# ComparativeGenomicsToolkit/cactus

Hardware: NVIDIA H100
Metric: BAR POA DP Gcells/sec and ends/sec at 1/2/4/8 H100 vs reference CPU BAR (higher is better)
Workload: dtype int32

## Files before the change

### cactus_b200/csrc/poa_cta.cuh

```cuda
#pragma once
#include <cuda_runtime.h>
#include "poa_graph.cuh"

namespace barb200 {

__device__ int cta_excl_scan(int *a, int n, int *ws) {
    const int T = blockDim.x, tid = threadIdx.x, lane = tid & 31, warp = tid >> 5, nw = T >> 5;
    const int chunk = (n + T - 1) / T, b = min(n, tid * chunk), e = min(n, b + chunk);
    int s = 0;
    for (int i = b; i < e; ++i) s += a[i];
    int inc = s;
#pragma unroll
    for (int off = 1; off < 32; off <<= 1) { const int v = __shfl_up_sync(0xffffffffu, inc, off); if (lane >= off) inc += v; }
    __syncthreads();
    if (lane == 31) ws[warp] = inc;
    __syncthreads();
    int woff = 0, total = 0;
    for (int k = 0; k < nw; ++k) { const int v = ws[k]; if (k < warp) woff += v; total += v; }
    int run = woff + inc - s;
    for (int i = b; i < e; ++i) { const int v = a[i]; a[i] = run; run += v; }
    __syncthreads();
    return total;
}

__device__ void cta_incl_max_scan(int *a, int n, int *ws) {
    const int T = blockDim.x, tid = threadIdx.x, lane = tid & 31, warp = tid >> 5, nw = T >> 5;
    const int chunk = (n + T - 1) / T, b = min(n, tid * chunk), e = min(n, b + chunk);
    int s = INT32_MIN;
    for (int i = b; i < e; ++i) s = max(s, a[i]);
    int inc = s;
#pragma unroll
    for (int off = 1; off < 32; off <<= 1) { const int v = __shfl_up_sync(0xffffffffu, inc, off); if (lane >= off) inc = max(inc, v); }
    int run = __shfl_up_sync(0xffffffffu, inc, 1);
    if (lane == 0) run = INT32_MIN;
    __syncthreads();
    if (lane == 31) ws[warp] = inc;
    __syncthreads();
    for (int k = 0; k < nw; ++k) if (k < warp) run = max(run, ws[k]);
    for (int i = b; i < e; ++i) { run = max(run, a[i]); a[i] = run; }
    __syncthreads();
}

__device__ __forceinline__ bool grow_in_par(Graph &g, int t) {
    if (g.in_n[t] < g.in_cap[t]) return true;
    const int ncap = g.in_cap[t] ? g.in_cap[t] * 2 : 2;
    const int noff = atomicAdd(&g.in_used, ncap);
    if (noff + ncap > g.in_pool) { g.err = JOB_ERR_EDGE_CAP; return false; }
    for (int i = 0; i < g.in_n[t]; ++i) { g.in_id[noff + i] = g.in_id[g.in_off[t] + i]; g.in_w[noff + i] = g.in_w[g.in_off[t] + i]; }
    g.in_off[t] = noff; g.in_cap[t] = ncap;
    return true;
}
__device__ __forceinline__ bool grow_out_par(Graph &g, int f) {
    if (g.out_n[f] < g.out_cap[f]) return true;
    const int ncap = g.out_cap[f] ? g.out_cap[f] * 2 : 2;
    const int noff = atomicAdd(&g.out_used, ncap);
    if (noff + ncap > g.out_pool) { g.err = JOB_ERR_EDGE_CAP; return false; }
    const int W = g.W;
    for (int i = 0; i < g.out_n[f]; ++i) {
        g.out_id[noff + i] = g.out_id[g.out_off[f] + i]; g.out_w[noff + i] = g.out_w[g.out_off[f] + i];
        for (int w = 0; w < W; ++w) g.out_rid[(int64_t)(noff + i) * W + w] = g.out_rid[(int64_t)(g.out_off[f] + i) * W + w];
    }
    for (int i = g.out_n[f]; i < ncap; ++i) for (int w = 0; w < W; ++w) g.out_rid[(int64_t)(noff + i) * W + w] = 0;
    g.out_off[f] = noff; g.out_cap[f] = ncap;
    return true;
}
__device__ __forceinline__ void graph_add_edge_par(Graph &g, int from, int to, int check_edge, int read_id) {
    int out_i = -1;
    if (check_edge) {
        const int io = g.in_off[to], in = g.in_n[to];
        for (int i = 0; i < in; ++i) if (g.in_id[io + i] == from) { g.in_w[io + i] += 1; break; }
        const int oo = g.out_off[from], on = g.out_n[from];
        for (int i = 0; i < on; ++i) if (g.out_id[oo + i] == to) { g.out_w[oo + i] += 1; out_i = i; break; }
    }
    if (out_i < 0) {
        if (!grow_in_par(g, to) || !grow_out_par(g, from)) return;
        const int ip = g.in_off[to] + g.in_n[to]; g.in_id[ip] = from; g.in_w[ip] = 1; g.in_n[to]++;
        out_i = g.out_n[from];
        const int op = g.out_off[from] + out_i; g.out_id[op] = to; g.out_w[op] = 1; g.out_n[from]++;
    }
    g.out_rid[(int64_t)(g.out_off[from] + out_i) * g.W + (read_id >> 6)] |= 1ULL << (read_id & 63);
}

__device__ void cta_add_first_sequence(Graph &g, const uint8_t *seq, int len, int read_id) {
    const int tid = threadIdx.x, T = blockDim.x, W = g.W;
    if (len + 2 > g.node_cap) { if (tid == 0) g.err = JOB_ERR_NODE_CAP; __syncthreads(); return; }
    if (2 * (len + 1) > g.in_pool || 2 * (len + 1) > g.out_pool) { if (tid == 0) g.err = JOB_ERR_EDGE_CAP; __syncthreads(); return; }
    const int rw = read_id >> 6; const uint64_t rb = 1ULL << (read_id & 63);
    for (int i = tid; i <= len; i += T) {
        const int to = i < len ? 2 + i : SINK_ID, from = i == 0 ? SRC_ID : 1 + i;
        g.in_off[to] = 2 * i; g.in_n[to] = 1; g.in_cap[to] = 2; g.in_id[2 * i] = from; g.in_w[2 * i] = 1;
        g.out_off[from] = 2 * i; g.out_n[from] = 1; g.out_cap[from] = 2; g.out_id[2 * i] = to; g.out_w[2 * i] = 1;
        for (int w = 0; w < W; ++w) { g.out_rid[(int64_t)(2 * i) * W + w] = w == rw ? rb : 0; g.out_rid[(int64_t)(2 * i + 1) * W + w] = 0; }
        if (i < len) { g.base[to] = seq[i]; g.aln_n[to] = 0; }
        g.index_to_node[i + 1] = to; g.node_to_index[to] = i + 1;
    }
    if (tid == 0) { g.index_to_node[0] = SRC_ID; g.node_to_index[SRC_ID] = 0; }
    if (tid == 0) { g.node_n = len + 2; g.in_used = 2 * (len + 1); g.out_used = 2 * (len + 1); }
    __syncthreads();
}

__device__ void cta_fuse_alignment(Graph &g, const uint8_t *seq, int L, const uint64_t *cigar, int n_cigar, int read_id, int *ws) {
    const int tid = threadIdx.x, T = blockDim.x;
    if (n_cigar == 0) return;
    int *node_of = g.tmp0, *is_new = g.tmp1;
    for (int c = tid; c < n_cigar; c += T) {
        const uint64_t cg = cigar[c];
        const int op = (int)(cg & 0xf);
        if (op == CMATCH) {
            const int node_id = (int)((cg >> 34) & 0x3fffffff), q = (int)((cg >> 4) & 0x3fffffff);
            const uint8_t b = seq[q];
            if (g.base[node_id] == b) { node_of[q] = node_id; is_new[q] = 0; }
            else {
                const int a = graph_aligned_with_base(g, node_id, b);
                if (a != -1) { node_of[q] = a; is_new[q] = 0; } else { node_of[q] = -1 - node_id; is_new[q] = 1; }
            }
        } else if (op == CINS) {
            const int qe = (int)((cg >> 34) & 0x3fffffff), len = (int)((cg >> 4) & 0x3fffffff);
            for (int q = qe - len + 1; q <= qe; ++q) { node_of[q] = INT32_MIN; is_new[q] = 1; }
        }
    }
    __syncthreads();
    const int first_new = g.node_n;
    const int n_new = cta_excl_scan(is_new, L, ws);
    if (first_new + n_new > g.node_cap) { if (tid == 0) g.err = JOB_ERR_NODE_CAP; __syncthreads(); return; }
    for (int q = tid; q < L; q += T) {
        const int m = node_of[q];
        if (m >= 0) { is_new[q] = 0; continue; }
        const int nid = first_new + is_new[q];
        g.base[nid] = seq[q]; g.aln_n[nid] = 0;
        g.in_off[nid] = 0; g.in_n[nid] = 0; g.in_cap[nid] = 0; g.out_off[nid] = 0; g.out_n[nid] = 0; g.out_cap[nid] = 0;
        if (m != INT32_MIN) graph_add_aligned(g, -1 - m, nid);
        node_of[q] = nid; is_new[q] = 1;
    }
    if (tid == 0) g.node_n = first_new + n_new;
    __syncthreads();
    if (g.err) return;
    {
        int *anc = g.remain, *cnt = g.msa_rank, *new_i2n = g.tmp1;
        const int n_old = first_new;
        for (int q = tid; q < L; q += T) {
            const int v = node_of[q];
            int e = v < first_new ? g.node_to_index[v] : -1;
            for (int k = 0; k < g.aln_n[v]; ++k) { const int a = g.aln_id[v * 4 + k]; if (a < first_new) e = max(e, g.node_to_index[a]); }
            anc[q] = e;
        }
        for (int i = tid; i < n_old; i += T) cnt[i] = 0;
        __syncthreads();
        cta_incl_max_scan(anc, L, ws);
        for (int q = tid; q < L; q += T) if (node_of[q] >= first_new) atomicAdd(&cnt[max(anc[q], 0)], 1);
        __syncthreads();
        cta_excl_scan(cnt, n_old, ws);
        for (int i = tid; i < n_old; i += T) new_i2n[i + cnt[i]] = g.index_to_node[i];
        for (int q = tid; q < L; q += T) { const int v = node_of[q]; if (v >= first_new) new_i2n[max(anc[q], 0) + 1 + (v - first_new)] = v; }
        __syncthreads();
        for (int k = tid; k < first_new + n_new; k += T) { const int v = new_i2n[k]; g.index_to_node[k] = v; g.node_to_index[v] = k; }
        __syncthreads();
    }
    for (int q = tid; q <= L; q += T) {
        const int from = q == 0 ? SRC_ID : node_of[q - 1], to = q == L ? SINK_ID : node_of[q];
        const int fresh = (q > 0 && from >= first_new) || (q < L && to >= first_new);
        graph_add_edge_par(g, from, to, fresh ? 0 : 1, read_id);
    }
    __syncthreads();
}


__device__ __forceinline__ void prefetch_l2(const void *p) { asm volatile("prefetch.global.L2 [%0];" ::"l"(p)); }

__device__ int warp_backtrack_step(const RowTables &rt, const DpState &d, const PoaParams &P, const int *smat8, const uint8_t *q,
                                   int &i, int &j, int &cur_op, int &len) {
    const unsigned FULLM = 0xffffffffu;
    const int lane = threadIdx.x & 31, inf = P.inf_min, e1 = P.e1, e2 = P.e2, oe1 = P.o1 + P.e1, oe2 = P.o2 + P.e2;
    len = 1;
    const RowRec rc = rt.rec[i];
    const RowInfo ri = d.info[i];
    const int *rowi = d.planes + d.row_off[i];
    const int npre = rc.base_npre >> 8;
    const int s = smat8[8 * (rc.base_npre & 0xff) + q[j - 1]];
    int hij = inf; unsigned cij = (unsigned)E_NEG16 | (unsigned)E_NEG16 << 16;
    if (j >= ri.beg && j <= ri.end) { hij = __ldcg(rowi + plane_index(ri.beg, ri.end, 0, j)); cij = (unsigned)__ldcg(rowi + plane_index(ri.beg, ri.end, 1, j)); }
    int hk0 = inf;
    if ((cur_op & OP_F) && j - 1 - lane >= ri.beg && j - 1 - lane <= ri.end) hk0 = __ldcg(rowi + plane_index(ri.beg, ri.end, 0, j - 1 - lane));
    int pi = -1, pm = inf, ph = inf, pe1 = inf, pe2 = inf; bool m_in = false, e_in = false;
    auto probe = [&](int kb) {
        const int k = kb + lane;
        pi = -1; m_in = false; e_in = false;
        if (k >= npre) return;
        pi = k == 0 ? rc.pre0 : rt.pre_row[rc.pre_off + k];
        const RowInfo pin = d.info[pi];
        const int *prow = d.planes + d.row_off[pi];
        m_in = (cur_op & OP_M) && j - 1 >= pin.beg && j - 1 <= pin.end;
        e_in = (cur_op & OP_E) && j >= pin.beg && j <= pin.end;
        if (m_in) pm = __ldcg(prow + plane_index(pin.beg, pin.end, 0, j - 1));
        if (e_in) {
            ph = __ldcg(prow + plane_index(pin.beg, pin.end, 0, j));
            const unsigned code = (unsigned)__ldcg(prow + plane_index(pin.beg, pin.end, 1, j));
            pe1 = e_decode(ph, (int)(code & 0xffffu), inf); pe2 = e_decode(ph, (int)(code >> 16), inf);
        }
    };
    if (cur_op & OP_M) {
        for (int kb = 0; kb < npre; kb += 32) {
            probe(kb);
            const unsigned hit = __ballot_sync(FULLM, m_in && pm + s == hij);
            if (hit) { i = __shfl_sync(FULLM, pi, __ffs(hit) - 1); --j; cur_op = OP_ALL; return CMATCH; }
        }
    }
    if (cur_op & OP_E) {
        const int own_e1 = e_decode(hij, (int)(cij & 0xffffu), inf), own_e2 = e_decode(hij, (int)(cij >> 16), inf);
        for (int kb = 0; kb < npre; kb += 32) {
            if (npre > 32 || !(cur_op & OP_M)) probe(kb);
            const bool ok1 = e_in && (cur_op & OP_E1) && ((cur_op & OP_M) ? hij == pe1 : own_e1 == pe1 - e1);
            const bool ok2 = e_in && (cur_op & OP_E2) && ((cur_op & OP_M) ? hij == pe2 : own_e2 == pe2 - e2);
            const unsigned hit = __ballot_sync(FULLM, ok1 || ok2);
            if (hit) {
                const int f = __ffs(hit) - 1;
                const int nop = ok1 ? ((ph - oe1 == pe1) ? (OP_M | OP_F) : OP_E1) : ((ph - oe2 == pe2) ? (OP_M | OP_F) : OP_E2);
                cur_op = __shfl_sync(FULLM, nop, f); i = __shfl_sync(FULLM, pi, f);
                return CDEL;
            }
        }
    }
    if (cur_op & OP_F) {
        if (!(cur_op & OP_M)) return -1;
        const int avail = j - ri.beg;
        int t1_max;
        if (e1 > e2) t1_max = oe2 >= oe1 ? (oe2 - oe1) / (e1 - e2) + 1 : 0;
        else t1_max = (e1 < e2 || oe1 <= oe2) ? avail : 0;
        if (t1_max > avail) t1_max = avail;
        for (int which = 0; which < 2; ++which) {
            if (!(cur_op & (which ? OP_F2 : OP_F1))) continue;
            const int oe = which ? oe2 : oe1, e = which ? e2 : e1, tmax = which ? avail : t1_max;
            for (int t0 = 0; t0 < tmax; t0 += 32) {
                const int t = t0 + lane + 1;
                int hk = hk0;
                if (t0 > 0) { hk = inf; if (t <= avail) hk = __ldcg(rowi + plane_index(ri.beg, ri.end, 0, j - t)); }
                const unsigned hit = __ballot_sync(FULLM, t <= tmax && hk == hij + oe + (t - 1) * e);
                if (hit) { len = __ffs(hit); len += t0; j -= len; cur_op = OP_M | OP_E; return CINS; }
            }
        }
    }
    return -1;
}

__device__ void warp_backtrack(Graph &g, const RowTables &rt, DpState &d, const PoaParams &P, const int *smat8, const uint8_t *q, int L) {
    const unsigned FULLM = 0xffffffffu;
    const int lane = threadIdx.x & 31, inf = P.inf_min;
    if (lane == 0) { dp_best_cell(g, rt, d, P, L); d.fc_row = -1; d.fc_hi = -1; }
    __syncwarp();
    int i = d.best_i, j = d.best_j, cur_op = OP_ALL, nc = 0, last_op = -1;
    uint64_t *cg = d.cigar; const int cap = d.cigar_cap;
    int fail = 0;
    auto push = [&](int op, int len, int node_id, int query_id) {
        if (nc == 0 || op != CINS || last_op != CINS) {
            if (nc >= cap) { fail = JOB_ERR_CIGAR_CAP; return; }
            if (lane == 0) {
                const uint64_t n_id = (uint64_t)(int64_t)node_id, q_id = (uint64_t)(int64_t)query_id, l = (uint64_t)len;
                cg[nc] = op == CMATCH ? (n_id << 34 | q_id << 4 | (uint64_t)op) : op == CINS ? (q_id << 34 | l << 4 | (uint64_t)op) : (n_id << 34 | l << 4 | (uint64_t)op);
            }
            ++nc;
        } else if (lane == 0) cg[nc - 1] += (uint64_t)len << 4;
        last_op = op;
    };
    if (j < L) push(CINS, L - j, -1, L - 1);
#ifdef BT_PROFILE
    long long pf_t0 = clock64(), pf_run_t = 0, pf_step_t = 0; int pf_iters = 0, pf_runs = 0, pf_cells = 0, pf_steps = 0, pf_ins = 0;
#endif
    while (i > 0 && j > 0 && !fail) {
        int run = 0;
#ifdef BT_PROFILE
        long long pf_a = clock64();
#endif
        if (cur_op == OP_ALL) {
            int c = i - lane, pre = -1, base = 0, n_ok = 0, node = 0;
            RowInfo ric; ric.beg = 0; ric.end = -1; ric.left = 0; ric.right = 0;
            int64_t ro = 0;
            bool fresh = true;
#pragma unroll 1
            for (int it = 0; it < 4; ++it) {
                if (fresh) {
                    pre = -1;
                    if (c > 0) { const RowRec rc = rt.rec[c]; base = rc.base_npre & 0xff; pre = (rc.base_npre >> 8) ? rc.pre0 : -1; node = g.index_to_node[c]; }
                    if (c >= 0) { ric = d.info[c]; ro = d.row_off[c]; }
                }
                const int nxt = __shfl_down_sync(FULLM, c, 1);
                const bool ok = lane < 31 && pre >= 0 && pre == nxt;
                n_ok = __ffs(~__ballot_sync(FULLM, ok)) - 1;
                if (n_ok >= 31 || it == 3) break;
                const int pre_b = __shfl_sync(FULLM, pre, n_ok);
                if (pre_b < 0) break;
                fresh = lane > n_ok;
                if (fresh) c = pre_b - (lane - n_ok - 1);
            }
            const int jj = j - lane;
            int hv = inf, inb = 0;
            if (lane <= n_ok && c >= 0 && jj >= 0) {
                inb = jj >= ric.beg && jj <= ric.end;
                if (inb) hv = __ldcg(d.planes + ro + plane_index(ric.beg, ric.end, 0, jj));
            }
            const int cl = c - 32, jl = jj - 32;
            RowInfo ril; ril.beg = 0; ril.end = -1; ril.left = 0; ril.right = 0;
            int64_t rol = 0;
            if (cl >= 0 && jl >= 0) { ril = d.info[cl]; rol = d.row_off[cl]; prefetch_l2(rt.rec + cl); prefetch_l2(g.index_to_node + cl); }
            const int h_next = __shfl_down_sync(FULLM, hv, 1), inb_next = __shfl_down_sync(FULLM, inb, 1);
            bool hit = false;
            if (lane < n_ok && c > 0 && jj >= 1 && inb_next) hit = h_next + smat8[8 * base + q[jj - 1]] == hv;
            run = __ffs(~__ballot_sync(FULLM, hit)) - 1;
            if (run > 0) {
                if (nc + run > cap) fail = JOB_ERR_CIGAR_CAP;
                else {
                    if (lane < run) cg[nc + lane] = (uint64_t)node << 34 | (uint64_t)(jj - 1) << 4 | (uint64_t)CMATCH;
                    nc += run; last_op = CMATCH;
                    i = __shfl_sync(FULLM, c, run); j -= run;
                }
            }
            if (cl >= 0 && jl >= 0 && jl <= ril.end) prefetch_l2(d.planes + rol + plane_index(ril.beg, ril.end, 0, jl < ril.beg ? ril.beg : jl));
        }
#ifdef BT_PROFILE
        long long pf_b = clock64(); if (cur_op == OP_ALL) { pf_run_t += pf_b - pf_a; ++pf_iters; if (run) { ++pf_runs; pf_cells += run; } }
#endif
        if (run == 0 && !fail) {
            const int id = g.index_to_node[i], jq = j - 1;
            int len = 1;
            const int op = warp_backtrack_step(rt, d, P, smat8, q, i, j, cur_op, len);
            if (op < 0) fail = JOB_ERR_BACKTRACK; else push(op, len, id, jq);
#ifdef BT_PROFILE
            pf_step_t += clock64() - pf_b; ++pf_steps; if (op == CINS) ++pf_ins;
#endif
        }
    }
#ifdef BT_PROFILE
    if (lane == 0 && blockIdx.x == 0) printf("bt L=%d total=%lld run_t=%lld step_t=%lld iters=%d runs=%d cells=%d steps=%d ins=%d\n", L, clock64() - pf_t0, pf_run_t, pf_step_t, pf_iters, pf_runs, pf_cells, pf_steps, pf_ins);
#endif
    if (!fail && j > 0) push(CINS, j, -1, j - 1);
    if (fail) { if (lane == 0) g.err = fail; return; }
    if (lane == 0) d.n_cigar = nc;
    __syncwarp();
    for (int a = lane; a < nc >> 1; a += 32) { const uint64_t t = cg[a]; cg[a] = cg[nc - 1 - a]; cg[nc - 1 - a] = t; }
    __syncwarp();
}

struct BfsScratch { uint32_t *optr; uint16_t *odst, *queue, *indeg; uint8_t *alnn; };

__device__ __forceinline__ size_t bfs_scratch_bytes(int n, int E) { return (size_t)4 * (n + 1) + (size_t)2 * E + 4 * (size_t)n + n + 16; }

__device__ void bfs_index_smem(Graph &g, const BfsScratch &B) {
    const int n = g.node_n;
    int head = 0, tail = 0;
    B.queue[tail++] = SRC_ID;
    while (head < tail) {
        const int cur = B.queue[head++];
        if (cur == SINK_ID) {
            if (head != n) g.err = JOB_ERR_TOPO;
            return;
        }
        const uint32_t o0 = B.optr[cur], o1 = B.optr[cur + 1];
        for (uint32_t i = o0; i < o1; ++i) {
            const int o = B.odst[i];
            const int left = (int)B.indeg[o] - 1; B.indeg[o] = (uint16_t)left;
            if (left == 0) {
                const int an = B.alnn[o];
                bool ok = true;
                for (int j = 0; j < an; ++j) if (B.indeg[g.aln_id[o * 4 + j]] != 0) { ok = false; break; }
                if (!ok) continue;
                B.queue[tail++] = (uint16_t)o;
                for (int j = 0; j < an; ++j) B.queue[tail++] = (uint16_t)g.aln_id[o * 4 + j];
            }
        }
    }
    g.err = JOB_ERR_TOPO;
}

__device__ void cta_topo_sort(Graph &g, RowTables &rt, unsigned char *scr, int scr_bytes, int *ws, bool have_order) {
    const int tid = threadIdx.x, T = blockDim.x, n = g.node_n;
    if (have_order) {
        for (int v = tid; v < n; v += T) graph_sort_node_edges(g, v);
        __syncthreads();
    } else {
    for (int v = tid; v < n; v += T) g.tmp0[v] = g.out_n[v];
    __syncthreads();
    const int E = cta_excl_scan(g.tmp0, n, ws);
    if (n < 65536 && bfs_scratch_bytes(n, E) <= (size_t)scr_bytes) {
        BfsScratch B;
        B.optr = reinterpret_cast<uint32_t *>(scr);
        B.odst = reinterpret_cast<uint16_t *>(B.optr + n + 1);
        B.queue = B.odst + E; B.indeg = B.queue + n;
        B.alnn = reinterpret_cast<uint8_t *>(B.indeg + n);
        for (int v = tid; v < n; v += T) {
            const uint32_t o = (uint32_t)g.tmp0[v];
            B.optr[v] = o;
            const int oo = g.out_off[v], on = g.out_n[v];
            for (int i = 0; i < on; ++i) B.odst[o + i] = (uint16_t)g.out_id[oo + i];
            B.indeg[v] = (uint16_t)g.in_n[v]; B.alnn[v] = g.aln_n[v];
        }
        if (tid == 0) B.optr[n] = (uint32_t)E;
        __syncthreads();
        if (T > 32) {
            if (tid == 0) bfs_index_smem(g, B);
            else if (tid >= 32) for (int v = tid - 32; v < n; v += T - 32) graph_sort_node_edges(g, v);
        } else {
            if (tid == 0) bfs_index_smem(g, B);
            __syncwarp();
            for (int v = tid; v < n; v += T) graph_sort_node_edges(g, v);
        }
        __syncthreads();
        if (g.err) return;
        for (int k = tid; k < n; k += T) { const int v = B.queue[k]; g.index_to_node[k] = v; g.node_to_index[v] = k; }
    } else {
        if (tid == 0) graph_bfs_index(g);
        __syncthreads();
        if (g.err) return;
        for (int v = tid; v < n; v += T) graph_sort_node_edges(g, v);
    }
    __syncthreads();
    }
    int *nx[2] = {g.tmp0, g.tmp1}, *dd[2] = {g.remain, g.msa_rank};
    for (int v = tid; v < n; v += T) {
        int nxt = SINK_ID, dist = 0;
        if (v != SINK_ID) {
            int max_w = -1;
            const int oo = g.out_off[v], on = g.out_n[v];
            for (int i = 0; i < on; ++i) if (g.out_w[oo + i] > max_w) { max_w = g.out_w[oo + i]; nxt = g.out_id[oo + i]; }
            dist = 1;
        }
        nx[0][v] = nxt; dd[0][v] = dist;
    }
    __syncthreads();
    int cur = 0;
    for (int span = 1; span < n; span <<= 1, cur ^= 1) {
        for (int v = tid; v < n; v += T) {
            const int nv = nx[cur][v];
            dd[cur ^ 1][v] = dd[cur][v] + dd[cur][nv];
            nx[cur ^ 1][v] = nx[cur][nv];
        }
        __syncthreads();
    }
    if (cur == 0) { for (int v = tid; v < n; v += T) g.remain[v] -= 1; }
    else { for (int v = tid; v < n; v += T) g.remain[v] = g.msa_rank[v] - 1; }
    __syncthreads();
    for (int r = tid; r < n; r += T) g.tmp0[r] = g.in_n[g.index_to_node[r]];
    __syncthreads();
    cta_excl_scan(g.tmp0, n, ws);
    for (int r = tid; r < n; r += T) graph_build_row(g, rt, r, g.tmp0[r]);
    __syncthreads();
}


__device__ void cta_msa_rank(Graph &g, unsigned char *scr, int scr_bytes, int *ws, int *msa_len_out) {
    const int tid = threadIdx.x, T = blockDim.x, n = g.node_n;
    for (int v = tid; v < n; v += T) g.tmp0[v] = g.out_n[v];
    __syncthreads();
    const int E = cta_excl_scan(g.tmp0, n, ws);
    if (n < 65535 && bfs_scratch_bytes(n, E) + 2 * (size_t)n <= (size_t)scr_bytes) {
        BfsScratch B;
        B.optr = reinterpret_cast<uint32_t *>(scr);
        B.odst = reinterpret_cast<uint16_t *>(B.optr + n + 1);
        B.queue = B.odst + E; B.indeg = B.queue + n;
        uint16_t *rk = B.indeg + n;
        B.alnn = reinterpret_cast<uint8_t *>(rk + n);
        for (int v = tid; v < n; v += T) {
            const uint32_t o = (uint32_t)g.tmp0[v];
            B.optr[v] = o;
            const int oo = g.out_off[v], on = g.out_n[v];
            for (int i = 0; i < on; ++i) B.odst[o + i] = (uint16_t)g.out_id[oo + i];
            B.indeg[v] = (uint16_t)g.in_n[v]; B.alnn[v] = g.aln_n[v];
        }
        if (tid == 0) B.optr[n] = (uint32_t)E;
        __syncthreads();
        if (tid == 0) {
            uint16_t *st = B.queue;
            int sp = 0, rank = 0, len = -1;
            st[sp++] = SRC_ID; rk[SRC_ID] = 0xffff;
            while (sp > 0) {
                const int cur = st[--sp];
                if (rk[cur] == 0xffff) {
                    rk[cur] = (uint16_t)rank;
                    for (int i = 0; i < B.alnn[cur]; ++i) rk[g.aln_id[cur * 4 + i]] = (uint16_t)rank;
                    ++rank;
                }
                if (cur == SINK_ID) { len = (int)rk[SINK_ID] - 1; break; }
                const uint32_t o0 = B.optr[cur], o1 = B.optr[cur + 1];
                for (uint32_t i = o0; i < o1; ++i) {
                    const int o = B.odst[i];
                    const int left = (int)B.indeg[o] - 1; B.indeg[o] = (uint16_t)left;
                    if (left == 0) {
                        const int an = B.alnn[o];
                        bool ok = true;
                        for (int j = 0; j < an; ++j) if (B.indeg[g.aln_id[o * 4 + j]] != 0) { ok = false; break; }
                        if (!ok) continue;
                        st[sp++] = (uint16_t)o; rk[o] = 0xffff;
                        for (int j = 0; j < an; ++j) { const int a = g.aln_id[o * 4 + j]; st[sp++] = (uint16_t)a; rk[a] = 0xffff; }
                    }
                }
            }
            if (len < 0) g.err = JOB_ERR_TOPO;
            *msa_len_out = len;
        }
        __syncthreads();
        if (g.err) return;
        for (int v = tid; v < n; v += T) g.msa_rank[v] = rk[v];
    } else {
        if (tid == 0) *msa_len_out = graph_msa_rank(g);
    }
    __syncthreads();
}

}
```

### cactus_b200/csrc/poa_kernel.cu

```cuda
#include <cuda_runtime.h>
#include <stdint.h>
#include "poa_graph.cuh"
#include "poa_cta.cuh"
#include "poa_kernel.cuh"

namespace barb200 {

#define FULL 0xffffffffu

struct KShared {
    Graph g; RowTables rt; DpState d;
    int job, msa_len_s, abort_s;
    __align__(256) int smat[5 * 8];
    int wF[2][2][32];
    int wM[2][4][32];
    RowRec rec[2];
    RowInfo ring_info[2];
};

__device__ __forceinline__ int4 ld4cg(const int *p) { return __ldcg(reinterpret_cast<const int4 *>(p)); }
__device__ __forceinline__ void st4(int *p, int a, int b, int c, int d) {
    asm volatile("st.global.v4.s32 [%0], {%1, %2, %3, %4};" ::"l"(p), "r"(a), "r"(b), "r"(c), "r"(d) : "memory");
}
__device__ __forceinline__ void sts4(unsigned a, int x, int y, int z, int w) {
    asm volatile("st.shared.v4.s32 [%0], {%1, %2, %3, %4};" ::"r"(a), "r"(x), "r"(y), "r"(z), "r"(w) : "memory");
}
__device__ __forceinline__ int4 lds4(unsigned a) {
    int4 v;
    asm volatile("ld.shared.v4.s32 {%0, %1, %2, %3}, [%4];" : "=r"(v.x), "=r"(v.y), "=r"(v.z), "=r"(v.w) : "r"(a) : "memory");
    return v;
}
__device__ __forceinline__ int lds1(unsigned a) {
    int v;
    asm volatile("ld.shared.s32 %0, [%1];" : "=r"(v) : "r"(a) : "memory");
    return v;
}
__device__ __forceinline__ int lds_const(unsigned a) {
    int v;
    asm("ld.shared.s32 %0, [%1];" : "=r"(v) : "r"(a));
    return v;
}
__device__ __forceinline__ int max3(int a, int b, int c) { return max(max(a, b), c); }
__device__ __forceinline__ void cp_async16(void *smem, const void *gmem) {
    asm volatile("cp.async.cg.shared.global [%0], [%1], 16;" ::"r"((unsigned)__cvta_generic_to_shared(smem)), "l"(gmem) : "memory");
}
__device__ __forceinline__ void cp_async_wait_all() { asm volatile("cp.async.wait_all;" ::: "memory"); }
__device__ __forceinline__ void store_pad(int *tp, int64_t cs, int NEG) {
#pragma unroll
    for (int c = 0; c < TB / CHUNK; ++c) st4(tp + c * cs, c < CPT / CHUNK ? NEG : 0, c < CPT / CHUNK ? NEG : 0, c < CPT / CHUNK ? NEG : 0, c < CPT / CHUNK ? NEG : 0);
}


template <bool MASKED>
__device__ __forceinline__ void row_pass1(int (&H)[CPT], int (&E1)[CPT], int (&E2)[CPT], unsigned mbase, const uint32_t (&qo)[4],
                                          int j0, int beg, int end, int NEG, int e1, int e2, int &agg1, int &agg2) {
#pragma unroll
    for (int e = 0; e < CPT; ++e) {
        const int s = lds_const(__byte_perm(qo[e >> 2], mbase, 0x7650 | (e & 3)));
        int h = __vimax3_s32(H[e] + s, E1[e], E2[e]);
        if (MASKED) {
            const bool inb = (unsigned)(j0 + e - beg) <= (unsigned)(end - beg);
            h = inb ? h : NEG; E1[e] = inb ? E1[e] : NEG; E2[e] = inb ? E2[e] : NEG;
        }
        H[e] = h;
    }
    int a1 = H[CPT - 1], a2 = H[CPT - 1];
#pragma unroll
    for (int e = CPT - 2; e >= 0; --e) { a1 = __viaddmax_s32(a1, e1, H[e]); a2 = __viaddmax_s32(a2, e2, H[e]); }
    agg1 = max(agg1, a1 + j0 * e1); agg2 = max(agg2, a2 + j0 * e2);
}

template <bool ROW0>
__device__ __forceinline__ void pred_chunk(int (&H)[CPT], int (&E1)[CPT], int (&E2)[CPT], int oc, int4 h4, int4 d4, int NEG) {
    const int h[CHUNK] = {h4.x, h4.y, h4.z, h4.w}, dv[CHUNK] = {d4.x, d4.y, d4.z, d4.w};
#pragma unroll
    for (int u = 0; u < CHUNK; ++u) {
        const int e = oc * CHUNK + u;
        const int c1 = dv[u] & 0xffff, c2 = (int)((unsigned)dv[u] >> 16);
        if (e + 1 < CPT) H[e + 1] = max(H[e + 1], h[u]);
        E1[e] = max(E1[e], ROW0 && c1 == E_NEG16 ? NEG : h[u] - c1); E2[e] = max(E2[e], ROW0 && c2 == E_NEG16 ? NEG : h[u] - c2);
    }
}

template <int MODE, int RING_NT>
__device__ __forceinline__ void row_pass2(int (&H)[CPT], int (&E1)[CPT], int (&E2)[CPT], int F1, int F2, int j0, int beg, int end, int NEG,
                                          int e1, int e2, int oe1, int oe2, int *tp, int64_t cs, unsigned rs, int &tmax) {
#pragma unroll
    for (int oc = 0; oc < CPT / CHUNK; ++oc) {
        int dd[CHUNK];
#pragma unroll
        for (int u = 0; u < CHUNK; ++u) {
            const int e = oc * CHUNK + u, hp = H[e];
            int h = __vimax3_s32(hp, F1, F2);
            F1 = __viaddmax_s32(F1, -e1, hp - oe1); F2 = __viaddmax_s32(F2, -e2, hp - oe2);
            int x1 = __viaddmax_s32(E1[e], -e1, h - oe1);
            int x2 = __viaddmax_s32(E2[e], -e2, h - oe2);
            if (MODE == 1) {
                const bool inb = (unsigned)(j0 + e - beg) <= (unsigned)(end - beg);
                h = inb ? h : NEG; x1 = inb ? x1 : NEG; x2 = inb ? x2 : NEG;
            } else if (MODE == 2) {
                const bool inb = j0 + e <= end;
                h = inb ? h : NEG; x1 = inb ? x1 : NEG; x2 = inb ? x2 : NEG;
            }
            H[e] = h; E1[e] = x1; E2[e] = x2;
            dd[u] = __byte_perm(h - x1, h - x2, 0x5410);
            tmax = max(tmax, h);
        }
        st4(tp + oc * cs, H[oc * CHUNK], H[oc * CHUNK + 1], H[oc * CHUNK + 2], H[oc * CHUNK + 3]);
        st4(tp + (CPT / CHUNK + oc) * cs, dd[0], dd[1], dd[2], dd[3]);
        if (RING_NT) {
            sts4(rs + oc * RING_NT * 16, H[oc * CHUNK], H[oc * CHUNK + 1], H[oc * CHUNK + 2], H[oc * CHUNK + 3]);
            sts4(rs + (CPT / CHUNK + oc) * RING_NT * 16, dd[0], dd[1], dd[2], dd[3]);
        }
    }
}

template <bool MASKED>
__device__ __forceinline__ void row_argmax(const int (&H)[CPT], int v, int j0, int beg, int end, int &tl, int &tr) {
    unsigned m = 0;
#pragma unroll
    for (int e = 0; e < CPT; ++e) m |= H[e] == v ? 1u << e : 0u;
    if (MASKED) {
        const int lo = max(beg - j0, 0), hi = min(end - j0, CPT - 1);
        m &= (2u << hi) - (1u << lo);
    }
    if (m) { tl = j0 + __ffs(m) - 1; tr = j0 + 31 - __clz(m); }
}

template <int NT>
__device__ long long dp_sweep(KShared &S, const BatchArgs &A, const uint8_t *__restrict__ qg, int L, uint4 *qsm, unsigned ring) {
    constexpr int RING_NT = poa_ring_bytes(NT) ? NT : 0;
    constexpr unsigned SLOT = NT * TB * sizeof(int), RCS = NT * 16;
    const int tid = threadIdx.x, lane = tid & 31, warp = tid >> 5, nwarps = NT >> 5;
    const unsigned my_ring = ring + tid * 16;
    const PoaParams &P = A.P;
    uint8_t *const sb = A.slots + (int64_t)blockIdx.x * A.lay.slot_bytes;
    const RowRec *const rec_tab = reinterpret_cast<const RowRec *>(sb + A.lay.o_row_rec);
    const int *const pre_row = reinterpret_cast<const int *>(sb + A.lay.o_pre_row);
    RowInfo *const info = reinterpret_cast<RowInfo *>(sb + A.lay.o_row_info);
    int64_t *const row_off = reinterpret_cast<int64_t *>(sb + A.lay.o_row_off);
    int *const planes = A.planes + (int64_t)blockIdx.x * A.lay.plane_cap;
    const int64_t plane_cap = A.lay.plane_cap;
    const int node_n = S.g.node_n, R = node_n - 1;
    const int NEG = P.inf_min, e1 = P.e1, e2 = P.e2, oe1 = P.o1 + P.e1, oe2 = P.o2 + P.e2;
    const int w = P.wb + (int)(P.wf * L);
    const int pn_shift = reference_lane_count(P, L, node_n) == 16 ? 4 : 3;
    static_assert(CPT == 16, "shifts below assume 16 columns per thread");
    const int j0 = tid * CPT;

    uint32_t qo[4] = {0u, 0u, 0u, 0u};
#pragma unroll
    for (int e = 0; e < CPT; ++e) {
        const int j = j0 + e;
        const uint32_t c = (j >= 1 && j <= L) ? qg[j - 1] : 5u;
        qo[e >> 2] |= (4u * c) << ((e & 3) * 8);
    }
    qsm[tid] = make_uint4(qo[0], qo[1], qo[2], qo[3]);
    const unsigned smat_s = (unsigned)__cvta_generic_to_shared(S.smat);

    int H[CPT], E1[CPT], E2[CPT];
    bool prev_active;
    int prev_beg = 0, prev_end, prev_left = 0, prev_right = 0;
    int cur_blk = 0, cells = 0;

    {
        const int dd = L - rec_tab[0].rd;
        prev_end = min(L, max(0, dd) + w);
        const int nT = prev_end / CPT + 1, nTs = row_blocks(0, prev_end);
        if ((int64_t)nTs * TB > plane_cap) return -1;
        prev_active = tid < nT;
        int D[CPT];
#pragma unroll
        for (int e = 0; e < CPT; ++e) {
            const int j = j0 + e;
            if (j == 0) { H[e] = 0; E1[e] = -oe1; E2[e] = -oe2; D[e] = oe1 | (oe2 << 16); }
            else if (j <= prev_end) { H[e] = max(-P.o1 - e1 * j, -P.o2 - e2 * j); E1[e] = NEG; E2[e] = NEG; D[e] = E_NEG16 | (E_NEG16 << 16); }
            else { H[e] = E1[e] = E2[e] = NEG; D[e] = 0; }
        }
        if (tid < nTs) {
            int *tp = planes + chunk_index(nTs, tid, 0);
            const int64_t cs = chunk_index(nTs, 0, 1);
#pragma unroll
            for (int oc = 0; oc < CPT / CHUNK; ++oc) {
                st4(tp + oc * cs, H[oc * CHUNK], H[oc * CHUNK + 1], H[oc * CHUNK + 2], H[oc * CHUNK + 3]);
                st4(tp + (CPT / CHUNK + oc) * cs, D[oc * CHUNK], D[oc * CHUNK + 1], D[oc * CHUNK + 2], D[oc * CHUNK + 3]);
            }
        }
        if (RING_NT) {
#pragma unroll
            for (int oc = 0; oc < CPT / CHUNK; ++oc) {
                sts4(my_ring + oc * RCS, H[oc * CHUNK], H[oc * CHUNK + 1], H[oc * CHUNK + 2], H[oc * CHUNK + 3]);
                sts4(my_ring + (CPT / CHUNK + oc) * RCS, D[oc * CHUNK], D[oc * CHUNK + 1], D[oc * CHUNK + 2], D[oc * CHUNK + 3]);
            }
        }
        if (lane == 31) S.wM[0][3][warp] = H[CPT - 1];
        if (tid == 0) {
            RowInfo ri; ri.beg = 0; ri.end = prev_end; ri.left = 0; ri.right = 0; info[0] = ri; row_off[0] = 0;
            if (RING_NT) S.ring_info[0] = ri;
        }
        cur_blk = nTs; cells = prev_end + 1;
        if (tid == 0) { cp_async16(&S.rec[1], rec_tab + (R > 1 ? 1 : 0)); cp_async_wait_all(); }
    }
    __syncthreads();

    for (int r = 1; r < R; ++r) {
        const int par = r & 1;
        const RowRec rec = S.rec[par];
        if (tid == 0 && r + 1 < R) cp_async16(&S.rec[par ^ 1], rec_tab + r + 1);
        const int b = rec.base_npre & 0xff, npre = rec.base_npre >> 8;
        const int dd = L - rec.rd;
        int maxL = node_n, maxR = 0, min_pre_beg = 0x7fffffff;
        bool has_prev = false;
        if (npre == 1 && rec.pre0 == r - 1) {
            maxL = min(node_n, prev_left + 1); maxR = prev_right + 1; min_pre_beg = prev_beg; has_prev = true;
        } else {
#pragma unroll 1
            for (int k = 0; k < npre; ++k) {
                const int p = k == 0 ? rec.pre0 : pre_row[rec.pre_off + k];
                int pl, pr, pb;
                if (p == r - 1) { pl = prev_left; pr = prev_right; pb = prev_beg; has_prev = true; }
                else if (RING_NT && p == r - 2) { const RowInfo pi = S.ring_info[par]; pl = pi.left; pr = pi.right; pb = pi.beg; }
                else { const RowInfo pi = info[p]; pl = pi.left; pr = pi.right; pb = pi.beg; }
                maxL = min(maxL, pl + 1); maxR = max(maxR, pr + 1); min_pre_beg = min(min_pre_beg, pb);
            }
        }
        const bool only_prev = npre == 1 && has_prev;
        int beg = max(0, min(maxL, dd) - w);
        const int end = min(L, max(maxR, dd) + w);
        if ((beg >> pn_shift) < (min_pre_beg >> pn_shift)) beg = min_pre_beg;
        const int t0 = beg >> 4, nT = (end >> 4) - t0 + 1, tt = tid - t0;
        const int nTs = row_blocks(beg, end), tts = tid - row_t0(beg);
        if ((int64_t)(cur_blk + nTs) * TB > plane_cap) return -1;
        const bool active = tt >= 0 && tt < nT;
        const int wmode = __any_sync(FULL, active && j0 < beg) ? 1 : __any_sync(FULL, active && j0 + CPT - 1 > end) ? 2 : 0;
        const uint32_t qadd = 0x01010101u * (32u * b);

        int hl = __shfl_up_sync(FULL, prev_active ? H[CPT - 1] : NEG, 1);
        if (lane == 0) hl = warp > 0 ? S.wM[par ^ 1][3][warp - 1] : NEG;

        const int id1 = NEG + beg * e1 + P.o1, id2 = NEG + beg * e2 + P.o2;
        int agg1 = id1, agg2 = id2;
        if (active) {
            if (has_prev && prev_active) {
#pragma unroll
                for (int e = CPT - 1; e >= 1; --e) H[e] = H[e - 1];
                H[0] = hl;
            } else {
#pragma unroll
                for (int e = 0; e < CPT; ++e) { H[e] = NEG; E1[e] = NEG; E2[e] = NEG; }
                if (has_prev) H[0] = hl;
            }
#pragma unroll 1
            for (int k = only_prev ? npre : 0; k < npre; ++k) {
                const int p = k == 0 ? rec.pre0 : pre_row[rec.pre_off + k];
                if (p == r - 1) continue;
                if (RING_NT && p == r - 2) {
                    const RowInfo pi = S.ring_info[par];
                    const int pt0 = pi.beg >> 4, pnT = (pi.end >> 4) - pt0 + 1, ptt = tid - pt0;
                    const unsigned rs = my_ring + par * SLOT;
                    if (ptt >= 0 && ptt < pnT) {
                        if (p == 0) {
#pragma unroll
                            for (int oc = 0; oc < CPT / CHUNK; ++oc) pred_chunk<true>(H, E1, E2, oc, lds4(rs + oc * RCS), lds4(rs + (CPT / CHUNK + oc) * RCS), NEG);
                        } else {
#pragma unroll
                            for (int oc = 0; oc < CPT / CHUNK; ++oc) pred_chunk<false>(H, E1, E2, oc, lds4(rs + oc * RCS), lds4(rs + (CPT / CHUNK + oc) * RCS), NEG);
                        }
                    }
                    if (ptt >= 1 && ptt <= pnT) H[0] = max(H[0], lds1(rs + (CPT / CHUNK - 1) * RCS - 4));
                    continue;
                }
                const RowInfo pi = info[p];
                const int pt0 = pi.beg >> 4, pnT = (pi.end >> 4) - pt0 + 1, ptt = tid - pt0, pnTs = row_blocks(pi.beg, pi.end);
                const int *Hp = planes + row_off[p] + chunk_index(pnTs, tid - row_t0(pi.beg), 0);
                const int64_t pcs = chunk_index(pnTs, 0, 1);
                if (ptt >= 0 && ptt < pnT) {
#pragma unroll
                    for (int oc = 0; oc < CPT / CHUNK; ++oc) pred_chunk<true>(H, E1, E2, oc, ld4cg(Hp + oc * pcs), ld4cg(Hp + (CPT / CHUNK + oc) * pcs), NEG);
                }
                if (ptt >= 1 && ptt <= pnT) H[0] = max(H[0], __ldcg(Hp - CHUNK + (CPT / CHUNK - 1) * pcs + CHUNK - 1));
            }
            const uint4 q4 = qsm[tid];
            const uint32_t qo[4] = {q4.x + qadd, q4.y + qadd, q4.z + qadd, q4.w + qadd};
            if (wmode != 1) row_pass1<false>(H, E1, E2, smat_s, qo, j0, beg, end, NEG, e1, e2, agg1, agg2);
            else row_pass1<true>(H, E1, E2, smat_s, qo, j0, beg, end, NEG, e1, e2, agg1, agg2);
        }
        int inc1 = agg1, inc2 = agg2;
#pragma unroll
        for (int off = 1; off < 32; off <<= 1) {
            const int n1 = __shfl_up_sync(FULL, inc1, off), n2 = __shfl_up_sync(FULL, inc2, off);
            if (lane >= off) { inc1 = max(inc1, n1); inc2 = max(inc2, n2); }
        }
        int ex1 = __shfl_up_sync(FULL, inc1, 1), ex2 = __shfl_up_sync(FULL, inc2, 1);
        if (lane == 0) { ex1 = id1; ex2 = id2; }
        if (lane == 31) { S.wF[par][0][warp] = inc1; S.wF[par][1][warp] = inc2; }
        __syncthreads();
        int P1, P2;
        {
            const int wv1 = lane < warp ? S.wF[par][0][lane] : id1, wv2 = lane < warp ? S.wF[par][1][lane] : id2;
            P1 = max(__reduce_max_sync(FULL, wv1), ex1); P2 = max(__reduce_max_sync(FULL, wv2), ex2);
        }
        int tmax = INT32_MIN;
        {
            int *tp = planes + (int64_t)cur_blk * TB + chunk_index(nTs, tts, 0);
            const int64_t cs = chunk_index(nTs, 0, 1);
            const unsigned rs = my_ring + par * SLOT;
            if (active) {
                const int F1 = P1 - P.o1 - j0 * e1, F2 = P2 - P.o2 - j0 * e2;
                if (wmode == 0) row_pass2<0, RING_NT>(H, E1, E2, F1, F2, j0, beg, end, NEG, e1, e2, oe1, oe2, tp, cs, rs, tmax);
                else if (wmode == 2) row_pass2<2, RING_NT>(H, E1, E2, F1, F2, j0, beg, end, NEG, e1, e2, oe1, oe2, tp, cs, rs, tmax);
                else row_pass2<1, RING_NT>(H, E1, E2, F1, F2, j0, beg, end, NEG, e1, e2, oe1, oe2, tp, cs, rs, tmax);
            } else if ((unsigned)tts < (unsigned)nTs) store_pad(tp, cs, NEG);
        }
        {
            const int wmax = __reduce_max_sync(FULL, tmax);
            int tleft = 0x7fffffff, tright = -1;
            if (active && tmax == wmax) {
                if (wmode == 0) row_argmax<false>(H, wmax, j0, beg, end, tleft, tright); else row_argmax<true>(H, wmax, j0, beg, end, tleft, tright);
            }
            const int wl = __reduce_min_sync(FULL, tleft), wr = __reduce_max_sync(FULL, tright);
            if (lane == 0) { S.wM[par][0][warp] = wmax; S.wM[par][1][warp] = wl; S.wM[par][2][warp] = wr; }
            if (lane == 31) S.wM[par][3][warp] = active ? H[CPT - 1] : NEG;
        }
        if (tid == 0) cp_async_wait_all();
        __syncthreads();
        {
            const int v = lane < nwarps ? S.wM[par][0][lane] : INT32_MIN;
            const int bmax = __reduce_max_sync(FULL, v);
            const int l = (lane < nwarps && v == bmax) ? S.wM[par][1][lane] : 0x7fffffff;
            const int rr = (lane < nwarps && v == bmax) ? S.wM[par][2][lane] : -1;
            prev_left = __reduce_min_sync(FULL, l); prev_right = __reduce_max_sync(FULL, rr);
        }
        prev_beg = beg; prev_end = end; prev_active = active;
        if (tid == 0) {
            RowInfo ri; ri.beg = beg; ri.end = end; ri.left = prev_left; ri.right = prev_right; info[r] = ri; row_off[r] = (int64_t)cur_blk * TB;
            if (RING_NT) S.ring_info[par] = ri;
        }
        cur_blk += nTs; cells += end - beg + 1;
    }
    __syncthreads();
    return cells;
}

__device__ __forceinline__ void carve(KShared &S, const BatchArgs &A, int slot) {
    const SlotLayout &Y = A.lay;
    uint8_t *b = A.slots + (int64_t)slot * Y.slot_bytes;
    Graph &g = S.g; RowTables &rt = S.rt; DpState &d = S.d;
    g.node_cap = Y.node_cap; g.in_pool = Y.in_pool; g.out_pool = Y.out_pool;
    g.base = b + Y.o_base; g.aln_n = b + Y.o_aln_n; g.aln_id = (int *)(b + Y.o_aln_id);
    g.in_off = (int *)(b + Y.o_in_off); g.in_n = (int *)(b + Y.o_in_n); g.in_cap = (int *)(b + Y.o_in_cap);
    g.out_off = (int *)(b + Y.o_out_off); g.out_n = (int *)(b + Y.o_out_n); g.out_cap = (int *)(b + Y.o_out_cap);
    g.in_id = (int *)(b + Y.o_in_id); g.in_w = (int *)(b + Y.o_in_w);
    g.out_id = (int *)(b + Y.o_out_id); g.out_w = (int *)(b + Y.o_out_w); g.out_rid = (uint64_t *)(b + Y.o_out_rid);
    g.index_to_node = (int *)(b + Y.o_index_to_node); g.node_to_index = (int *)(b + Y.o_node_to_index);
    g.remain = (int *)(b + Y.o_remain); g.msa_rank = (int *)(b + Y.o_msa_rank);
    g.tmp0 = (int *)(b + Y.o_tmp0); g.tmp1 = (int *)(b + Y.o_tmp1);
    rt.rec = (RowRec *)(b + Y.o_row_rec); rt.pre_row = (int *)(b + Y.o_pre_row);
    d.planes = A.planes + (int64_t)slot * Y.plane_cap; d.plane_cap = Y.plane_cap;
    d.row_off = (int64_t *)(b + Y.o_row_off); d.info = (RowInfo *)(b + Y.o_row_info);
    d.cigar = (uint64_t *)(b + Y.o_cigar); d.cigar_cap = Y.cigar_cap; d.n_cigar = 0;
    d.fc = (int *)(b + Y.o_fc); d.fc_cap = Y.fc_cap; d.fc_row = -1; d.fc_hi = -1;
}

#define PHASE_TICK(ph) do { if (A.phase_clk && threadIdx.x == 0) { unsigned long long _n = clock64(); A.phase_clk[(size_t)blockIdx.x * PH_N + (ph)] += _n - t_last; t_last = _n; } } while (0)

template <int NT>
__device__ __forceinline__ void poa_msa_body(const BatchArgs &A) {
    extern __shared__ __align__(16) unsigned char dyn_smem[];
    __shared__ KShared S;
    __shared__ uint4 qsm[NT];
    const int tid = threadIdx.x;
    int *ws = &S.wF[0][0][0];
    if (tid == 0) carve(S, A, blockIdx.x);
    for (int k = tid; k < 40; k += blockDim.x) S.smat[k] = (k & 7) < 5 ? A.P.mat[(k >> 3) * 5 + (k & 7)] : 0;
    unsigned long long t_last = A.phase_clk ? clock64() : 0ULL, t_start = t_last;
    __syncthreads();

    while (true) {
        if (tid == 0) {
            const int k = atomicAdd(A.next_job, 1);
            int j = -1;
            if (k < A.n_jobs) j = A.job_base + k;
            S.job = j;
        }
        __syncthreads();
        const int job = S.job;
        if (job < 0) break;
        const JobDesc jd = A.jobs[job];
        const int K = jd.n_seq;
        const int *lens = A.lens + jd.len_off;
        const int64_t *soff = A.soff + jd.len_off;
        const uint8_t *seqs = A.seqs + jd.seq_off;
        if (tid == 0) { graph_reset(S.g, K); S.abort_s = 0; }
        __syncthreads();
        const int *const order = A.order + jd.len_off;
        if (tid == 0 && A.gt_status[job]) S.g.err = JOB_ERR_GT_CAP;
        __syncthreads();
        long long cells = 0;
        for (int a = 0; a < K && !S.g.err; ++a) {
            const int read = order[a], L = lens[read];
            const uint8_t *q = seqs + soff[read];
            if (a == 0) {
                if (A.serial_phases) { if (tid == 0) graph_add_first_sequence(S.g, q, L, read); }
                else cta_add_first_sequence(S.g, q, L, read);
                PHASE_TICK(PH_FUSE);
            } else {
                long long c = -2;
                if (L + 1 <= CPT * (int)blockDim.x) c = dp_sweep<NT>(S, A, q, L, qsm, (unsigned)__cvta_generic_to_shared(dyn_smem));
                if (c < 0) { if (tid == 0) S.g.err = c == -2 ? JOB_ERR_QUERY_LEN : JOB_ERR_PLANE_CAP; c = 0; }
                cells += c;
                __syncthreads();
                PHASE_TICK(PH_DP);
                if (A.serial_phases) { if (tid == 0 && !S.g.err) { dp_best_cell(S.g, S.rt, S.d, A.P, L); dp_backtrack(S.g, S.rt, S.d, A.P, q, L); } }
                else if (tid < 32 && !S.g.err) warp_backtrack(S.g, S.rt, S.d, A.P, S.smat, q, L);
                PHASE_TICK(PH_BACKTRACK);
                __syncthreads();
                if (A.serial_phases) { if (tid == 0 && !S.g.err) graph_fuse_alignment(S.g, q, S.d.cigar, S.d.n_cigar, read); }
                else if (!S.g.err) cta_fuse_alignment(S.g, q, L, S.d.cigar, S.d.n_cigar, read, ws);
                PHASE_TICK(PH_FUSE);
            }
            __syncthreads();
            if (S.g.err) break;
            if (A.serial_phases) { if (tid == 0) graph_topo_sort_serial(S.g, S.rt); __syncthreads(); }
            else cta_topo_sort(S.g, S.rt, dyn_smem, A.scratch_bytes, ws, A.bfs_order == 0);
            PHASE_TICK(PH_TOPO);
            if (S.g.err) break;
        }
        __syncthreads();
        if (!S.g.err) {
            if (A.serial_phases) { if (tid == 0) S.msa_len_s = graph_msa_rank(S.g); __syncthreads(); }
            else cta_msa_rank(S.g, dyn_smem, A.scratch_bytes, ws, &S.msa_len_s);
            if (tid == 0 && !S.g.err && S.msa_len_s > jd.msa_stride) S.g.err = JOB_ERR_MSA_CAP;
        }
        __syncthreads();
        if (!S.g.err) {
            const int ml = S.msa_len_s;
            uint8_t *msa = A.msa + jd.msa_off;
            for (int64_t i = tid; i < (int64_t)K * ml; i += blockDim.x) msa[(i / ml) * jd.msa_stride + (i % ml)] = GAP_CODE;
            __syncthreads();
            for (int v = 2 + tid; v < S.g.node_n; v += blockDim.x) graph_msa_fill_node(S.g, v, msa, jd.msa_stride);
        }
        __syncthreads();
        if (tid == 0) { A.status[job] = S.g.err; A.msa_len[job] = S.g.err ? 0 : S.msa_len_s; A.cells[job] = cells; }
        PHASE_TICK(PH_MSA);
        __syncthreads();
    }
    if (A.phase_clk && tid == 0) A.phase_clk[(size_t)blockIdx.x * PH_N + PH_TOTAL] += clock64() - t_start;
}

extern "C" __global__ void __launch_bounds__(32, 16) poa_msa_kernel_t32(const BatchArgs A) { poa_msa_body<32>(A); }
extern "C" __global__ void __launch_bounds__(64, 8) poa_msa_kernel_t64(const BatchArgs A) { poa_msa_body<64>(A); }
#ifndef BARB200_T128_MINB
#define BARB200_T128_MINB 4
#endif
extern "C" __global__ void __launch_bounds__(128, BARB200_T128_MINB) poa_msa_kernel_t128(const BatchArgs A) { poa_msa_body<128>(A); }
extern "C" __global__ void __launch_bounds__(256, 2) poa_msa_kernel_t256(const BatchArgs A) { poa_msa_body<256>(A); }
extern "C" __global__ void __launch_bounds__(640, 1) poa_msa_kernel_t640(const BatchArgs A) { poa_msa_body<640>(A); }
extern "C" __global__ void __launch_bounds__(1024, 1) poa_msa_kernel_t1024(const BatchArgs A) { poa_msa_body<1024>(A); }

}
```

Before: 223.4.

## Stage topo-sort pointer jumping and fuse scratch arrays in shared memory

When the dynamic shared scratch is large enough, the pointer-jumping distance computation in topo sort now runs on 16-bit arrays in shared memory instead of global tmp buffers. Row tables are then built from a shared node-to-index map and an exclusive scan of in-degrees, and the function returns early. The fuse-alignment reorder arrays (anc, cnt, new_i2n) are likewise placed in shared scratch. Both changes aim to cut global memory traffic in the serial-per-read graph phases, at the cost of 16-bit limits and a second code path that must match the global version exactly.

```diff
diff --git a/cactus_b200/csrc/poa_cta.cuh b/cactus_b200/csrc/poa_cta.cuh
--- a/cactus_b200/csrc/poa_cta.cuh
+++ b/cactus_b200/csrc/poa_cta.cuh
@@ -99,7 +99,8 @@
     __syncthreads();
 }
 
-__device__ void cta_fuse_alignment(Graph &g, const uint8_t *seq, int L, const uint64_t *cigar, int n_cigar, int read_id, int *ws) {
+__device__ void cta_fuse_alignment(Graph &g, const uint8_t *seq, int L, const uint64_t *cigar, int n_cigar, int read_id,
+                                   unsigned char *scr, int scr_bytes, int *ws) {
     const int tid = threadIdx.x, T = blockDim.x;
     if (n_cigar == 0) return;
     int *node_of = g.tmp0, *is_new = g.tmp1;
@@ -136,8 +137,11 @@
     __syncthreads();
     if (g.err) return;
     {
+        const int n_old = first_new;
         int *anc = g.remain, *cnt = g.msa_rank, *new_i2n = g.tmp1;
-        const int n_old = first_new;
+        if ((size_t)4 * (L + 2 * n_old + n_new) <= (size_t)scr_bytes) {
+            anc = reinterpret_cast<int *>(scr); cnt = anc + L; new_i2n = cnt + n_old;
+        }
         for (int q = tid; q < L; q += T) {
             const int v = node_of[q];
             int e = v < first_new ? g.node_to_index[v] : -1;
@@ -370,10 +374,34 @@
     g.err = JOB_ERR_TOPO;
 }
 
+__device__ __forceinline__ int first_heaviest_out(const Graph &g, int v) {
+    int nxt = SINK_ID, max_w = -1;
+    const int oo = g.out_off[v], on = g.out_n[v];
+    for (int i = 0; i < on; ++i) if (g.out_w[oo + i] > max_w) { max_w = g.out_w[oo + i]; nxt = g.out_id[oo + i]; }
+    return nxt;
+}
+
+__device__ __forceinline__ void build_row_smem(const Graph &g, RowTables &rt, int r, int off, const uint16_t *n2i, const uint16_t *dist) {
+    const int v = g.index_to_node[r];
+    const int io = g.in_off[v], in = g.in_n[v];
+    int pre0 = -1;
+    for (int k = 0; k < in; ++k) { const int p = n2i[g.in_id[io + k]]; rt.pre_row[off + k] = p; if (k == 0) pre0 = p; }
+    RowRec rec;
+    rec.base_npre = g.base[v] | (in << 8);
+    rec.rd = (int)dist[v] - (int)dist[SINK_ID] - 1;
+    rec.pre_off = off;
+    rec.pre0 = pre0;
+    rt.rec[r] = rec;
+}
+
 __device__ void cta_topo_sort(Graph &g, RowTables &rt, unsigned char *scr, int scr_bytes, int *ws, bool have_order) {
     const int tid = threadIdx.x, T = blockDim.x, n = g.node_n;
+    const int np = (n + 1) & ~1;
+    const bool smem = n < 65536 && (size_t)8 * np <= (size_t)scr_bytes;
+    uint16_t *const s16 = reinterpret_cast<uint16_t *>(scr);
+    auto init_jump = [&](int v) { s16[v] = (uint16_t)first_heaviest_out(g, v); s16[2 * np + v] = v != SINK_ID; };
     if (have_order) {
-        for (int v = tid; v < n; v += T) graph_sort_node_edges(g, v);
+        for (int v = tid; v < n; v += T) { graph_sort_node_edges(g, v); if (smem) init_jump(v); }
         __syncthreads();
     } else {
     for (int v = tid; v < n; v += T) g.tmp0[v] = g.out_n[v];
@@ -412,6 +440,33 @@
         for (int v = tid; v < n; v += T) graph_sort_node_edges(g, v);
     }
     __syncthreads();
+    if (smem) {
+        for (int v = tid; v < n; v += T) init_jump(v);
+        __syncthreads();
+    }
+    }
+    if (smem) {
+        int cur = 0;
+        for (int span = 1; span < n; span <<= 1, cur ^= 1) {
+            const uint16_t *nx = s16 + cur * np, *dd = s16 + (2 + cur) * np;
+            uint16_t *nx_to = s16 + (cur ^ 1) * np, *dd_to = s16 + (2 + (cur ^ 1)) * np;
+            for (int v = tid; v < n; v += T) {
+                const int nv = nx[v];
+                dd_to[v] = (uint16_t)(dd[v] + dd[nv]);
+                nx_to[v] = nx[nv];
+            }
+            __syncthreads();
+        }
+        const uint16_t *dist = s16 + (2 + cur) * np;
+        for (int v = tid; v < n; v += T) g.remain[v] = (int)dist[v] - 1;
+        int *off = reinterpret_cast<int *>(scr);
+        uint16_t *n2i = s16 + (2 + (cur ^ 1)) * np;
+        for (int r = tid; r < n; r += T) { const int v = g.index_to_node[r]; n2i[v] = (uint16_t)r; off[r] = g.in_n[v]; }
+        __syncthreads();
+        cta_excl_scan(off, n, ws);
+        for (int r = tid; r < n; r += T) build_row_smem(g, rt, r, off[r], n2i, dist);
+        __syncthreads();
+        return;
     }
     int *nx[2] = {g.tmp0, g.tmp1}, *dd[2] = {g.remain, g.msa_rank};
     for (int v = tid; v < n; v += T) {
diff --git a/cactus_b200/csrc/poa_kernel.cu b/cactus_b200/csrc/poa_kernel.cu
--- a/cactus_b200/csrc/poa_kernel.cu
+++ b/cactus_b200/csrc/poa_kernel.cu
@@ -416,7 +416,7 @@
                 PHASE_TICK(PH_BACKTRACK);
                 __syncthreads();
                 if (A.serial_phases) { if (tid == 0 && !S.g.err) graph_fuse_alignment(S.g, q, S.d.cigar, S.d.n_cigar, read); }
-                else if (!S.g.err) cta_fuse_alignment(S.g, q, L, S.d.cigar, S.d.n_cigar, read, ws);
+                else if (!S.g.err) cta_fuse_alignment(S.g, q, L, S.d.cigar, S.d.n_cigar, read, dyn_smem, A.scratch_bytes, ws);
                 PHASE_TICK(PH_FUSE);
             }
             __syncthreads();
```

New measurement: 228.4 (median of 6 runs). +2.3%, better.
